# HaokunChen245/FedDAT

Hardware: AMD Instinct MI355X
Metric: VQA samples/sec, ViLT-B/32 dual-adapter local step (higher is better)
Workload: dtype fp16; 1 GPU; configs[1] with fp16 operands (BASELINE.json's configs[1] string says bf16: same operand width and MFMA rate; the bf16 step is in other_operand_format with --full): ViLT-B/32 FedDAT, 1 client per MI355X, fp16 MFMA operands (dynamic loss scale, GradScaler semantics on the device, initial 2^14), fp32 accumulate / masters, batch=32/client, 384x384 synthetic + 40-token questions, MKD on; batch_per_client=32, seq_len=185, clients=1, hip_graph=True, ranks=1, hetero_steps=False

## Files before the change

feddat_amd/csrc/adapter.hip:

```cpp
#include <type_traits>

#include "common.hip.h"

namespace {

constexpr int H = 768, R = 48, NT = 3, KS = H / 32, CT = H / 16;
constexpr int WCOLS = H / 4;
constexpr int WCH = WCOLS / 4;
constexpr int NLD = 16 * WCH / 64;
constexpr int ROWF = 200;
constexpr int STG_WAVE = 16 * ROWF;

struct AdapterLaunch {
    feddat_adapter_seg seg[2];
    int nseg;
    int tiles0;
};

#define FD_COMPILER_FENCE() asm volatile("" ::: "memory")

__device__ __forceinline__ void slice_load(const float* __restrict__ src, int nvalid, int lane, f32x4 (&v)[NLD]) {
#pragma unroll
    for (int j = 0; j < NLD; ++j) {
        const int f = j * 64 + lane, r = f / WCH, c = f - r * WCH;
        const int rr = r < nvalid ? r : nvalid - 1;
        v[j] = *reinterpret_cast<const f32x4*>(src + (size_t)rr * H + c * 4);
    }
}
__device__ __forceinline__ void slice_to_lds(float* stg, int lane, const f32x4 (&v)[NLD]) {
#pragma unroll
    for (int j = 0; j < NLD; ++j) {
        const int f = j * 64 + lane, r = f / WCH, c = f - r * WCH;
        *reinterpret_cast<f32x4*>(stg + r * ROWF + c * 4) = v[j];
    }
}
__device__ __forceinline__ void frags_from_lds(const float* stg, int lane, f32x4 (&keep)[KS / 4][2]) {
    const float* p = stg + (lane & 15) * ROWF + 4 * (lane >> 4);
#pragma unroll
    for (int k = 0; k < KS / 4; ++k) {
        keep[k][0] = *reinterpret_cast<const f32x4*>(p + k * 32);
        keep[k][1] = *reinterpret_cast<const f32x4*>(p + k * 32 + 16);
    }
}
__device__ __forceinline__ void frags_to_lds(float* stg, int lane, const f32x4 (&keep)[KS / 4][2]) {
    float* p = stg + (lane & 15) * ROWF + 4 * (lane >> 4);
#pragma unroll
    for (int k = 0; k < KS / 4; ++k) {
        *reinterpret_cast<f32x4*>(p + k * 32) = keep[k][0];
        *reinterpret_cast<f32x4*>(p + k * 32 + 16) = keep[k][1];
    }
}

template <int NA>
__device__ __forceinline__ void down_proj(const bf16* const* w, int lane, int ks0, f32x4 (&z)[2][NT],
                                          const f32x4 (&keep)[KS / 4][2]) {
#pragma unroll
    for (int k = 0; k < KS / 4; ++k) {
        const int q = ks0 + k;
        const bf16x8 xf = cvt8(keep[k][0], keep[k][1]);
#pragma unroll
        for (int a = 0; a < NA; ++a)
#pragma unroll
            for (int nt = 0; nt < NT; ++nt) {
                const bf16x8 wf = *reinterpret_cast<const bf16x8*>(w[a] + ((nt * KS + q) * 64 + lane) * 8);
                z[a][nt] = mfma16x32(wf, xf, z[a][nt]);
            }
    }
}

__device__ __forceinline__ void load_w48(const bf16* w, int ct, int lane, bf16x8& w01, bf16x8& w2) {
    w01 = *reinterpret_cast<const bf16x8*>(w + (ct * 64 + lane) * 8);
    const bf16x4 c = *reinterpret_cast<const bf16x4*>(w + CT * 64 * 8 + (ct * 64 + lane) * 4);
    w2 = bf16x8{c[0], c[1], c[2], c[3], 0, 0, 0, 0};
}
__device__ __forceinline__ bf16x8 pad8(const f32x4 a) {
    return bf16x8{(bf16)a[0], (bf16)a[1], (bf16)a[2], (bf16)a[3], 0, 0, 0, 0};
}

template <int NS>
__device__ __forceinline__ void ksplit_store(float* stg_all, int wave, int lane, int s, const f32x4 v) {
    reinterpret_cast<f32x4*>(stg_all + wave * STG_WAVE)[s * 64 + lane] = v;
}
template <int NS>
__device__ __forceinline__ f32x4 ksplit_sum(const float* stg_all, int lane, int s) {
    f32x4 t = reinterpret_cast<const f32x4*>(stg_all)[s * 64 + lane];
#pragma unroll
    for (int w = 1; w < 4; ++w) t = t + reinterpret_cast<const f32x4*>(stg_all + w * STG_WAVE)[s * 64 + lane];
    return t;
}

struct LnFuse {
    const float* gamma;
    const float* beta;
    bf16* y16;
    float* stats;
    float eps;
};

template <int NA, bool ZS>
__device__ __forceinline__ void bwd_body(const float* __restrict__ x, const float* __restrict__ dy,
                                         float* __restrict__ dx, bf16* __restrict__ dx16, float* __restrict__ z_out,
                                         float* __restrict__ dz_out, const feddat_adapter_seg& sg, int row0,
                                         float* stg_all, const float* __restrict__ z_saved) {
    const int lane = threadIdx.x & 63, wave = threadIdx.x >> 6;
    const int g = lane >> 4, i16 = lane & 15;
    const int nvalid = (sg.row_end - row0) < 16 ? (sg.row_end - row0) : 16;
    const bool valid = i16 < nvalid;
    const int row = row0 + i16;
    float* stg = stg_all + wave * STG_WAVE;

    const bf16* wd[2] = {(const bf16*)sg.wd[0], (const bf16*)sg.wd[NA - 1]};
    const bf16* wuT[2] = {(const bf16*)sg.wuT[0], (const bf16*)sg.wuT[NA - 1]};
    f32x4 z[2][NT], gr[2][NT];
#pragma unroll
    for (int a = 0; a < 2; ++a)
#pragma unroll
        for (int nt = 0; nt < NT; ++nt) {
            z[a][nt] = f32x4{0.f, 0.f, 0.f, 0.f};
            gr[a][nt] = f32x4{0.f, 0.f, 0.f, 0.f};
        }
    f32x4 dyk[KS / 4][2];
    f32x4 vd[NLD];
    if (ZS) {
        slice_load(dy + (size_t)row0 * H + wave * WCOLS, nvalid, lane, vd);
        const float* zrow = z_saved + (size_t)(valid ? row : row0 + nvalid - 1) * (2 * R) + 4 * g;
#pragma unroll
        for (int a = 0; a < NA; ++a)
#pragma unroll
            for (int nt = 0; nt < NT; ++nt) z[a][nt] = *reinterpret_cast<const f32x4*>(zrow + a * R + nt * 16);
        FD_COMPILER_FENCE();
    } else {
        f32x4 vx[NLD];
        slice_load(x + (size_t)(row0 + sg.x_row_delta) * H + wave * WCOLS, nvalid, lane, vx);
        FD_COMPILER_FENCE();
        f32x4 xk[KS / 4][2];
        slice_to_lds(stg, lane, vx);
        slice_load(dy + (size_t)row0 * H + wave * WCOLS, nvalid, lane, vd);
        FD_COMPILER_FENCE();
        frags_from_lds(stg, lane, xk);
        down_proj<NA>(wd, lane, wave * (KS / 4), z, xk);
    }
    slice_to_lds(stg, lane, vd);
    frags_from_lds(stg, lane, dyk);
    down_proj<NA>(wuT, lane, wave * (KS / 4), gr, dyk);
#pragma unroll
    for (int a = 0; a < NA; ++a)
#pragma unroll
        for (int nt = 0; nt < NT; ++nt) {
            if (!ZS) ksplit_store<2 * NA * NT>(stg_all, wave, lane, a * NT + nt, z[a][nt]);
            ksplit_store<2 * NA * NT>(stg_all, wave, lane, NA * NT + a * NT + nt, gr[a][nt]);
        }
    __syncthreads();

    bf16x8 dzb01[NA], dzb2[NA];
    f32x4 z_keep = f32x4{0.f, 0.f, 0.f, 0.f}, dz_keep = z_keep;
#pragma unroll
    for (int a = 0; a < NA; ++a) {
        const float sc = sg.scale[a];
#pragma unroll
        for (int nt = 0; nt < NT; ++nt) {
            const f32x4 gs = ksplit_sum<2 * NA * NT>(stg_all, lane, NA * NT + a * NT + nt);
            f32x4 zz, dz;
            if (ZS) {
                zz = z[a][nt];
            } else {
                const f32x4 zs = ksplit_sum<2 * NA * NT>(stg_all, lane, a * NT + nt);
                const f32x4 b4 = *reinterpret_cast<const f32x4*>(sg.bd[a] + nt * 16 + 4 * g);
#pragma unroll
                for (int e = 0; e < 4; ++e) zz[e] = fmaxf(zs[e] + b4[e], 0.f);
            }
#pragma unroll
            for (int e = 0; e < 4; ++e) dz[e] = zz[e] > 0.f ? sc * gs[e] : 0.f;
            gr[a][nt] = dz;
            if (a == sg.train_slot && nt == wave) {
                z_keep = zz;
                dz_keep = dz;
            }
        }
        dzb01[a] = cvt8(gr[a][0], gr[a][1]);
        dzb2[a] = pad8(gr[a][2]);
    }
    const bool export_z = sg.train_slot >= 0 && wave < NT && valid && z_out;

    if (dx) {
#pragma unroll
        for (int k = 0; k < CT / 4; ++k) {
            const int ct = wave * (CT / 4) + k;
            f32x4 o = dyk[k >> 1][k & 1];
#pragma unroll
            for (int a = 0; a < NA; ++a) {
                bf16x8 w01, w2;
                load_w48((const bf16*)sg.wdT[a], ct, lane, w01, w2);
                f32x4 y = mfma16x32(w01, dzb01[a], f32x4{0.f, 0.f, 0.f, 0.f});
                y = mfma16x32(w2, dzb2[a], y);
                o = o + y;
            }
            dyk[k >> 1][k & 1] = o;
        }
        __syncthreads();
        frags_to_lds(stg, lane, dyk);
    }
    if (export_z) {
        *reinterpret_cast<f32x4*>(z_out + (size_t)row * R + wave * 16 + 4 * g) = z_keep;
        *reinterpret_cast<f32x4*>(dz_out + (size_t)row * R + wave * 16 + 4 * g) = dz_keep;
    }
    if (!dx) return;
    float* orow = dx + (size_t)row0 * H + wave * WCOLS;
    f32x4 v[NLD];
#pragma unroll
    for (int j = 0; j < NLD; ++j) {
        const int f = j * 64 + lane, r = f / WCH, c = f - r * WCH;
        v[j] = *reinterpret_cast<const f32x4*>(stg + r * ROWF + c * 4);
    }
#pragma unroll
    for (int j = 0; j < NLD; ++j) {
        const int f = j * 64 + lane, r = f / WCH, c = f - r * WCH;
        if (r < nvalid) *reinterpret_cast<f32x4*>(orow + (size_t)r * H + c * 4) = v[j];
    }
    if (dx16) {
        bf16* brow = dx16 + (size_t)row0 * H + wave * WCOLS;
#pragma unroll
        for (int j = 0; j < NLD; ++j) {
            const int f = j * 64 + lane, r = f / WCH, c = f - r * WCH;
            if (r < nvalid) *reinterpret_cast<bf16x4*>(brow + (size_t)r * H + c * 4) = cvt4(v[j]);
        }
    }
}

template <bool ZS>
__global__ __launch_bounds__(256, 2) void adapter_bwd_kernel(const float* __restrict__ x, const float* __restrict__ dy,
                                                          float* __restrict__ dx, bf16* __restrict__ dx16,
                                                          float* __restrict__ z_out, float* __restrict__ dz_out,
                                                          AdapterLaunch L, const float* __restrict__ z_saved) {
    __shared__ __attribute__((aligned(16))) float stg[4 * STG_WAVE];
    const int tile = blockIdx.x;
    const int s = tile < L.tiles0 ? 0 : 1;
    const int t = s ? tile - L.tiles0 : tile;
    const feddat_adapter_seg& sg = L.seg[s];
    const int row0 = sg.row_begin + t * 16;
    if (sg.n_adapters == 2) bwd_body<2, ZS>(x, dy, dx, dx16, z_out, dz_out, sg, row0, stg, z_saved);
    else bwd_body<1, ZS>(x, dy, dx, dx16, z_out, dz_out, sg, row0, stg, z_saved);
}

constexpr int ROWT = H + 8;
constexpr int TILE_F = 16 * ROWT;
constexpr int KSPL_F = 4 * 6 * 64 * 4;
constexpr int ZT_F = 16 * 2 * R;

struct WsLaunch {
    AdapterLaunch a;
    int g0;
    int dbg;
};

#define FD_WAIT_VM0() asm volatile("s_waitcnt vmcnt(0)" ::: "memory")
constexpr int WS_WEIGHT_LOADS_PER_ADAPTER = NT * (KS / 4) + CT / 4 + 2 * (CT / 8);
static_assert(WS_WEIGHT_LOADS_PER_ADAPTER == 42, "ws_load_weights changed: re-derive the counted wait");
template <int NA>
__device__ __forceinline__ void ws_wait_tile0(bool has_tile1) {
    constexpr int behind = NA * WS_WEIGHT_LOADS_PER_ADAPTER + 12;
    constexpr int cnt = behind < 63 ? behind : 63;
    if (has_tile1) asm volatile("s_waitcnt vmcnt(%0)" ::"n"(cnt) : "memory");
    else FD_WAIT_VM0();
}

__device__ __forceinline__ void ws_dma16(const float* g, const float* lds_dst) {
    const unsigned a = __builtin_amdgcn_readfirstlane((unsigned)(uintptr_t)LDS_PTR(lds_dst));
    asm volatile("s_mov_b32 m0, %1\n\ts_nop 0\n\tglobal_load_lds_dwordx4 %0, off" : : "v"(g), "s"(a) : "memory");
}
__device__ __forceinline__ void ws_tile_dma(const float* __restrict__ src, int nvalid, float* buf, int wave, int lane) {
#pragma unroll
    for (int j = 0; j < 12; ++j) {
        const int r = wave * 4 + j / 3, part = j % 3;
        const int rr = r < nvalid ? r : nvalid - 1;
        ws_dma16(src + (size_t)rr * H + part * 256 + lane * 4, buf + r * ROWT + part * 256);
    }
}
__device__ __forceinline__ void ws_frags_from_lds(const float* buf, int wave, int lane, f32x4 (&keep)[KS / 4][2]) {
    const float* p = buf + (lane & 15) * ROWT + wave * WCOLS + 4 * (lane >> 4);
#pragma unroll
    for (int k = 0; k < KS / 4; ++k) {
        keep[k][0] = *reinterpret_cast<const f32x4*>(p + k * 32);
        keep[k][1] = *reinterpret_cast<const f32x4*>(p + k * 32 + 16);
    }
}
__device__ __forceinline__ void ws_frags_to_lds(float* buf, int wave, int lane, const f32x4 (&keep)[KS / 4][2]) {
    float* p = buf + (lane & 15) * ROWT + wave * WCOLS + 4 * (lane >> 4);
#pragma unroll
    for (int k = 0; k < KS / 4; ++k) {
        *reinterpret_cast<f32x4*>(p + k * 32) = keep[k][0];
        *reinterpret_cast<f32x4*>(p + k * 32 + 16) = keep[k][1];
    }
}

template <int NA>
struct WsWeights {
    bf16x8 dn[NA][NT][KS / 4];
    bf16x8 up01[NA][CT / 4];
    bf16x8 up2[NA][CT / 8];
};
template <int NA>
__device__ __forceinline__ void ws_load_weights(WsWeights<NA>& W, const void* const* dn, const void* const* up, int wave,
                                                int lane) {
#pragma unroll
    for (int a = 0; a < NA; ++a) {
        const bf16* d = (const bf16*)dn[a];
        const bf16* u = (const bf16*)up[a];
#pragma unroll
        for (int nt = 0; nt < NT; ++nt)
#pragma unroll
            for (int k = 0; k < KS / 4; ++k)
                W.dn[a][nt][k] = *reinterpret_cast<const bf16x8*>(d + ((nt * KS + wave * (KS / 4) + k) * 64 + lane) * 8);
#pragma unroll
        for (int k = 0; k < CT / 4; ++k) {
            const int ct = wave * (CT / 4) + k;
            W.up01[a][k] = *reinterpret_cast<const bf16x8*>(u + (ct * 64 + lane) * 8);
        }
#pragma unroll
        for (int p = 0; p < CT / 8; ++p) {
            const int ct = wave * (CT / 4) + 2 * p;
            const bf16x4 lo = *reinterpret_cast<const bf16x4*>(u + CT * 64 * 8 + (ct * 64 + lane) * 4);
            const bf16x4 hi = *reinterpret_cast<const bf16x4*>(u + CT * 64 * 8 + ((ct + 1) * 64 + lane) * 4);
            W.up2[a][p] = bf16x8{lo[0], lo[1], lo[2], lo[3], hi[0], hi[1], hi[2], hi[3]};
        }
    }
}
__device__ __forceinline__ bf16x8 pad8hi(const f32x4 a) {
    return bf16x8{0, 0, 0, 0, (bf16)a[0], (bf16)a[1], (bf16)a[2], (bf16)a[3]};
}

__device__ __forceinline__ void ws_walk(const WsLaunch& L, int& s, int& t0, int& tstep, int& ntiles) {
    const int b = blockIdx.x;
    s = b < L.g0 ? 0 : 1;
    t0 = s ? b - L.g0 : b;
    tstep = s ? (int)gridDim.x - L.g0 : L.g0;
    const feddat_adapter_seg& sg = L.a.seg[s];
    ntiles = (sg.row_end - sg.row_begin + 15) / 16;
}

template <int NA>
__device__ __forceinline__ void ws_fwd_body(const float* __restrict__ x, float* __restrict__ out,
                                            const feddat_adapter_seg& sg, int t0, int tstep, int ntiles, float* smem,
                                            const LnFuse& ln, float* __restrict__ z_save, const int dbg) {
    const int lane = threadIdx.x & 63, wave = threadIdx.x >> 6;
    const int g = lane >> 4, i16 = lane & 15;
    float* kspl = smem + 2 * TILE_F;
    float* lnred = kspl + KSPL_F;
    float* sbu = lnred + 256;
    float* sbd = sbu + 2 * H;
    float* sgam = sbd + 128;
    float* sbet = sgam + H;
    if (t0 >= ntiles) return;

    auto tile_dma = [&](int p) {
        const int t = t0 + p * tstep;
        if (t < ntiles && !(p && (dbg & 4))) {
            const int row0 = sg.row_begin + t * 16;
            const int nvalid = (sg.row_end - row0) < 16 ? (sg.row_end - row0) : 16;
            ws_tile_dma(x + (size_t)(row0 + sg.x_row_delta) * H, nvalid, smem + p * TILE_F, wave, lane);
        }
    };
    for (int i = threadIdx.x; i < NA * H; i += 256) sbu[i] = sg.bu[i / H][i % H];
    if (threadIdx.x < NA * R) sbd[(threadIdx.x / R) * 64 + threadIdx.x % R] = sg.bd[threadIdx.x / R][threadIdx.x % R];
    if (ln.gamma)
        for (int i = threadIdx.x; i < H; i += 256) {
            sgam[i] = ln.gamma[i];
            sbet[i] = ln.beta[i];
        }
    float sc[NA];
#pragma unroll
    for (int a = 0; a < NA; ++a) sc[a] = sg.scale[a];
    tile_dma(0);
    WsWeights<NA> W;
    ws_load_weights<NA>(W, sg.wd, sg.wu, wave, lane);
    tile_dma(1);
    ws_wait_tile0<NA>(!(dbg & 4) && t0 + tstep < ntiles);
    __syncthreads();

    int cur = 0;
    for (int t = t0; t < ntiles; t += tstep, cur ^= 1) {
        const int row0 = sg.row_begin + t * 16;
        const int nvalid = (sg.row_end - row0) < 16 ? (sg.row_end - row0) : 16;
        float* buf = smem + cur * TILE_F;

        f32x4 z_keep[NA];
        float mean = 0.f, rstd = 0.f;
#pragma unroll
        for (int a = 0; a < NA; ++a) z_keep[a] = f32x4{0.f, 0.f, 0.f, 0.f};
        if (!(dbg & 2)) {
        const float* frag = buf + i16 * ROWT + wave * WCOLS + 4 * g;
        f32x4 z[NA][NT];
#pragma unroll
        for (int a = 0; a < NA; ++a)
#pragma unroll
            for (int nt = 0; nt < NT; ++nt) z[a][nt] = f32x4{0.f, 0.f, 0.f, 0.f};
#pragma unroll
        for (int k = 0; k < KS / 4; ++k) {
            const bf16x8 xf = cvt8(*reinterpret_cast<const f32x4*>(frag + k * 32),
                                   *reinterpret_cast<const f32x4*>(frag + k * 32 + 16));
#pragma unroll
            for (int a = 0; a < NA; ++a)
#pragma unroll
                for (int nt = 0; nt < NT; ++nt) z[a][nt] = mfma16x32(W.dn[a][nt][k], xf, z[a][nt]);
        }
#pragma unroll
        for (int a = 0; a < NA; ++a)
#pragma unroll
            for (int nt = 0; nt < NT; ++nt)
                reinterpret_cast<f32x4*>(kspl)[(wave * 6 + a * NT + nt) * 64 + lane] = z[a][nt];
        __syncthreads();
        bf16x8 zb01[NA], zb2[NA][2];
#pragma unroll
        for (int a = 0; a < NA; ++a) {
#pragma unroll
            for (int nt = 0; nt < NT; ++nt) {
                f32x4 tsum = reinterpret_cast<const f32x4*>(kspl)[(a * NT + nt) * 64 + lane];
#pragma unroll
                for (int w = 1; w < 4; ++w) tsum = tsum + reinterpret_cast<const f32x4*>(kspl)[(w * 6 + a * NT + nt) * 64 + lane];
                const f32x4 b4 = *reinterpret_cast<const f32x4*>(sbd + a * 64 + nt * 16 + 4 * g);
#pragma unroll
                for (int e = 0; e < 4; ++e) z[a][nt][e] = fmaxf(tsum[e] + b4[e], 0.f);
                if (nt == wave) z_keep[a] = z[a][nt];
            }
            zb01[a] = cvt8(z[a][0], z[a][1]);
            zb2[a][0] = pad8(z[a][2]);
            zb2[a][1] = pad8hi(z[a][2]);
        }

        f32x4 xk[KS / 4][2];
#pragma unroll
        for (int k = 0; k < CT / 4; ++k) {
            const int c = (wave * (CT / 4) + k) * 16 + 4 * g;
            f32x4 o = *reinterpret_cast<const f32x4*>(frag + k * 16);
#pragma unroll
            for (int a = 0; a < NA; ++a) {
                f32x4 y = mfma16x32(W.up01[a][k], zb01[a], f32x4{0.f, 0.f, 0.f, 0.f});
                y = mfma16x32(W.up2[a][k >> 1], zb2[a][k & 1], y);
                const f32x4 bu4 = *reinterpret_cast<const f32x4*>(sbu + a * H + c);
#pragma unroll
                for (int e = 0; e < 4; ++e) o[e] += sc[a] * (y[e] + bu4[e]);
            }
            xk[k >> 1][k & 1] = o;
        }

        if (ln.gamma) {
            float s1 = 0.f;
#pragma unroll
            for (int k = 0; k < CT / 4; ++k) {
                const f32x4 o = xk[k >> 1][k & 1];
                s1 += (o[0] + o[1]) + (o[2] + o[3]);
            }
            s1 += __shfl_xor(s1, 16, 64);
            s1 += __shfl_xor(s1, 32, 64);
            const float mw = s1 * (1.0f / WCOLS);
            float s2 = 0.f;
#pragma unroll
            for (int k = 0; k < CT / 4; ++k)
#pragma unroll
                for (int e = 0; e < 4; ++e) {
                    const float d = xk[k >> 1][k & 1][e] - mw;
                    s2 += d * d;
                }
            s2 += __shfl_xor(s2, 16, 64);
            s2 += __shfl_xor(s2, 32, 64);
            if (g == 0) {
                lnred[wave * 32 + 2 * i16] = mw;
                lnred[wave * 32 + 2 * i16 + 1] = s2;
            }
            __syncthreads();
            const float m0 = lnred[2 * i16], m1 = lnred[32 + 2 * i16], m2 = lnred[64 + 2 * i16], m3 = lnred[96 + 2 * i16];
            mean = ((m0 + m1) + (m2 + m3)) * 0.25f;
            const float q0 = m0 - mean, q1 = m1 - mean, q2 = m2 - mean, q3 = m3 - mean;
            const float M2 = ((lnred[2 * i16 + 1] + lnred[32 + 2 * i16 + 1]) + (lnred[64 + 2 * i16 + 1] + lnred[96 + 2 * i16 + 1])) +
                             (float)WCOLS * ((q0 * q0 + q1 * q1) + (q2 * q2 + q3 * q3));
            rstd = rsqrtf(M2 * (1.0f / H) + ln.eps);
            if (g == 0) {
                lnred[128 + wave * 32 + 2 * i16] = mean;
                lnred[128 + wave * 32 + 2 * i16 + 1] = rstd;
            }
        }

        ws_frags_to_lds(buf, wave, lane, xk);
        }
        float* orow = out + (size_t)row0 * H + wave * WCOLS;
        const float* srow = buf + wave * WCOLS;
        f32x4 v[NLD];
#pragma unroll
        for (int j = 0; j < NLD; ++j) {
            const int r = 4 * (j / 3) + g, c = 16 * (j % 3) + i16;
            v[j] = *reinterpret_cast<const f32x4*>(srow + r * ROWT + c * 4);
        }
        FD_WAIT_VM0();
        const bool st_on = !(dbg & 1);
        auto emit = [&](auto full_tag) {
            constexpr bool FULL = decltype(full_tag)::value;
            if (z_save && wave < NT && (FULL || i16 < nvalid)) {
#pragma unroll
                for (int a = 0; a < NA; ++a)
                    *reinterpret_cast<f32x4*>(z_save + (size_t)(row0 + i16) * (2 * R) + a * R + wave * 16 + 4 * g) = z_keep[a];
            }
#pragma unroll
            for (int j = 0; j < NLD; ++j) {
                const int r = 4 * (j / 3) + g, c = 16 * (j % 3) + i16;
                if (FULL || r < nvalid) *reinterpret_cast<f32x4*>(orow + (size_t)r * H + c * 4) = v[j];
            }
            if (ln.gamma) {
                bf16* yrow = ln.y16 + (size_t)row0 * H + wave * WCOLS;
#pragma unroll
                for (int j = 0; j < NLD; ++j) {
                    const int r = 4 * (j / 3) + g, c = 16 * (j % 3) + i16;
                    const float m = lnred[128 + wave * 32 + 2 * r], rs = lnred[128 + wave * 32 + 2 * r + 1];
                    const f32x4 gm = *reinterpret_cast<const f32x4*>(sgam + wave * WCOLS + c * 4);
                    const f32x4 bt = *reinterpret_cast<const f32x4*>(sbet + wave * WCOLS + c * 4);
                    f32x4 y;
#pragma unroll
                    for (int e = 0; e < 4; ++e) y[e] = (v[j][e] - m) * rs * gm[e] + bt[e];
                    if (FULL || r < nvalid) *reinterpret_cast<bf16x4*>(yrow + (size_t)r * H + c * 4) = cvt4(y);
                }
                if (wave == 0 && g == 0 && (FULL || i16 < nvalid) && ln.stats) {
                    ln.stats[2 * (size_t)(row0 + i16)] = mean;
                    ln.stats[2 * (size_t)(row0 + i16) + 1] = rstd;
                }
            }
        };
        if (st_on) {
            if (nvalid == 16) emit(std::true_type{});
            else emit(std::false_type{});
        }
        __syncthreads();
        if (t + 2 * tstep < ntiles && !(dbg & 4)) {
            const int rn = sg.row_begin + (t + 2 * tstep) * 16;
            const int nv = (sg.row_end - rn) < 16 ? (sg.row_end - rn) : 16;
            ws_tile_dma(x + (size_t)(rn + sg.x_row_delta) * H, nv, buf, wave, lane);
        }
    }
}

constexpr int WS_FWD_LDS = (2 * TILE_F + KSPL_F + 256 + 2 * H + 128 + 2 * H) * 4;

__global__ __launch_bounds__(256, 1) void adapter_fwd_ws_kernel(const float* __restrict__ x, float* __restrict__ out,
                                                                WsLaunch L, LnFuse ln, float* __restrict__ z_save) {
    extern __shared__ __attribute__((aligned(16))) float ws_smem[];
    int s, t0, tstep, ntiles;
    ws_walk(L, s, t0, tstep, ntiles);
    const feddat_adapter_seg& sg = L.a.seg[s];
    if (sg.n_adapters == 2) ws_fwd_body<2>(x, out, sg, t0, tstep, ntiles, ws_smem, ln, z_save, FD_ABL(L.dbg));
    else ws_fwd_body<1>(x, out, sg, t0, tstep, ntiles, ws_smem, ln, z_save, FD_ABL(L.dbg));
}


__device__ __forceinline__ void ws_ztile_dma(const float* __restrict__ zs, int nvalid, float* dst, int wave, int lane) {
#pragma unroll
    for (int j = 0; j < 2; ++j) {
        const int piece = wave + 4 * j;
        if (piece < 6) {
            const int fo = piece * 256 + lane * 4, r = fo / (2 * R), c = fo - r * (2 * R);
            const int rr = r < nvalid ? r : nvalid - 1;
            ws_dma16(zs + (size_t)rr * (2 * R) + c, dst + piece * 256);
        }
    }
}

template <int NA, bool Q8>
__device__ __forceinline__ void ws_bwd_body(const float* __restrict__ dy, float* __restrict__ dx, bf16* __restrict__ dx16,
                                            float* __restrict__ z_out, float* __restrict__ dz_out,
                                            const feddat_adapter_seg& sg, int t0, int tstep, int ntiles, float* smem,
                                            const float* __restrict__ z_saved, const int dbg,
                                            unsigned char* __restrict__ dx8, float* __restrict__ dx8_scale) {
    const int lane = threadIdx.x & 63, wave = threadIdx.x >> 6;
    const int g = lane >> 4, i16 = lane & 15;
    float* kspl = smem + 2 * TILE_F;
    float* ztile = kspl + KSPL_F;
    float* amred = ztile + 2 * ZT_F;
    if (t0 >= ntiles) return;
    auto tile_dma = [&](int p) {
        const int t = t0 + p * tstep;
        if (t < ntiles && !(p && (dbg & 4))) {
            const int row0 = sg.row_begin + t * 16;
            const int nvalid = (sg.row_end - row0) < 16 ? (sg.row_end - row0) : 16;
            ws_tile_dma(dy + (size_t)row0 * H, nvalid, smem + p * TILE_F, wave, lane);
            ws_ztile_dma(z_saved + (size_t)row0 * (2 * R), nvalid, ztile + p * ZT_F, wave, lane);
        }
    };
    if (Q8) {
#pragma unroll
        for (int p = 0; p < 2; ++p) {
            const int t = t0 + p * tstep;
            if (t < ntiles && !(p && (dbg & 4))) {
                const int row0 = sg.row_begin + t * 16;
                const int nvalid = (sg.row_end - row0) < 16 ? (sg.row_end - row0) : 16;
                ws_tile_dma(dy + (size_t)row0 * H, nvalid, smem + p * TILE_F, wave, lane);
                ws_ztile_dma(z_saved + (size_t)row0 * (2 * R), nvalid, ztile + p * ZT_F, wave, lane);
            }
        }
    } else {
        tile_dma(0);
    }
    WsWeights<NA> W;
    ws_load_weights<NA>(W, sg.wuT, sg.wdT, wave, lane);
    if (!Q8) tile_dma(1);
    float sc[NA];
#pragma unroll
    for (int a = 0; a < NA; ++a) sc[a] = sg.scale[a];
    const int train_slot = sg.train_slot;
    const bool exp_z = train_slot >= 0 && wave < NT && z_out;
    ws_wait_tile0<NA>(!Q8 && !(dbg & 4) && t0 + tstep < ntiles);
    __syncthreads();

    int cur = 0;
    for (int t = t0; t < ntiles; t += tstep, cur ^= 1) {
        const int row0 = sg.row_begin + t * 16;
        const int nvalid = (sg.row_end - row0) < 16 ? (sg.row_end - row0) : 16;
        float* buf = smem + cur * TILE_F;
        float* zt = ztile + cur * ZT_F;

        f32x4 z_keep = f32x4{0.f, 0.f, 0.f, 0.f}, dz_keep = z_keep;
        if (!(dbg & 2)) {
        const float* frag = buf + i16 * ROWT + wave * WCOLS + 4 * g;
        f32x4 gr[NA][NT];
#pragma unroll
        for (int a = 0; a < NA; ++a)
#pragma unroll
            for (int nt = 0; nt < NT; ++nt) gr[a][nt] = f32x4{0.f, 0.f, 0.f, 0.f};
#pragma unroll
        for (int k = 0; k < KS / 4; ++k) {
            const bf16x8 df = cvt8(*reinterpret_cast<const f32x4*>(frag + k * 32),
                                   *reinterpret_cast<const f32x4*>(frag + k * 32 + 16));
#pragma unroll
            for (int a = 0; a < NA; ++a)
#pragma unroll
                for (int nt = 0; nt < NT; ++nt) gr[a][nt] = mfma16x32(W.dn[a][nt][k], df, gr[a][nt]);
        }
#pragma unroll
        for (int a = 0; a < NA; ++a)
#pragma unroll
            for (int nt = 0; nt < NT; ++nt)
                reinterpret_cast<f32x4*>(kspl)[(wave * 6 + a * NT + nt) * 64 + lane] = gr[a][nt];
        __syncthreads();

        bf16x8 dzb01[NA], dzb2[NA][2];
#pragma unroll
        for (int a = 0; a < NA; ++a) {
#pragma unroll
            for (int nt = 0; nt < NT; ++nt) {
                f32x4 gs = reinterpret_cast<const f32x4*>(kspl)[(a * NT + nt) * 64 + lane];
#pragma unroll
                for (int w = 1; w < 4; ++w) gs = gs + reinterpret_cast<const f32x4*>(kspl)[(w * 6 + a * NT + nt) * 64 + lane];
                const f32x4 zz = *reinterpret_cast<const f32x4*>(zt + i16 * (2 * R) + a * R + nt * 16 + 4 * g);
                f32x4 dz;
#pragma unroll
                for (int e = 0; e < 4; ++e) dz[e] = zz[e] > 0.f ? sc[a] * gs[e] : 0.f;
                gr[a][nt] = dz;
                if (a == train_slot && nt == wave) {
                    z_keep = zz;
                    dz_keep = dz;
                }
            }
            dzb01[a] = cvt8(gr[a][0], gr[a][1]);
            dzb2[a][0] = pad8(gr[a][2]);
            dzb2[a][1] = pad8hi(gr[a][2]);
        }
        if (dx) {
#pragma unroll
            for (int k = 0; k < CT / 4; ++k) {
                f32x4 o = *reinterpret_cast<const f32x4*>(frag + k * 16);
#pragma unroll
                for (int a = 0; a < NA; ++a) {
                    f32x4 y = mfma16x32(W.up01[a][k], dzb01[a], f32x4{0.f, 0.f, 0.f, 0.f});
                    y = mfma16x32(W.up2[a][k >> 1], dzb2[a][k & 1], y);
                    o = o + y;
                }
                *reinterpret_cast<f32x4*>(buf + i16 * ROWT + wave * WCOLS + 4 * g + k * 16) = o;
            }
        }
        }
        f32x4 v[NLD];
        if (dx) {
            const float* srow = buf + wave * WCOLS;
#pragma unroll
            for (int j = 0; j < NLD; ++j) {
                const int r = 4 * (j / 3) + g, c = 16 * (j % 3) + i16;
                v[j] = *reinterpret_cast<const f32x4*>(srow + r * ROWT + c * 4);
            }
        }
        float sc8[4] = {1.f, 1.f, 1.f, 1.f};
        if (Q8 && dx && dx8) {
#pragma unroll
            for (int q = 0; q < 4; ++q) {
                float am = 0.f;
#pragma unroll
                for (int jj = 0; jj < 3; ++jj)
#pragma unroll
                    for (int e = 0; e < 4; ++e) am = fmaxf(am, fabsf(v[3 * q + jj][e]));
                am = fmaxf(am, __shfl_xor(am, 1, 64));
                am = fmaxf(am, __shfl_xor(am, 2, 64));
                am = fmaxf(am, __shfl_xor(am, 4, 64));
                am = fmaxf(am, __shfl_xor(am, 8, 64));
                if (i16 == 0) amred[wave * 16 + 4 * q + g] = am;
            }
            __syncthreads();
#pragma unroll
            for (int q = 0; q < 4; ++q) {
                const int r = 4 * q + g;
                const float am = fmaxf(fmaxf(amred[r], amred[16 + r]), fmaxf(amred[32 + r], amred[48 + r]));
                sc8[q] = am > 0.f ? am * (1.0f / 448.0f) : 1.0f;
            }
        }
        FD_WAIT_VM0();
        const bool st_on = !(dbg & 1);
        auto emit = [&](auto full_tag) {
            constexpr bool FULL = decltype(full_tag)::value;
            if (exp_z && (FULL || i16 < nvalid)) {
                *reinterpret_cast<f32x4*>(z_out + (size_t)(row0 + i16) * R + wave * 16 + 4 * g) = z_keep;
                *reinterpret_cast<f32x4*>(dz_out + (size_t)(row0 + i16) * R + wave * 16 + 4 * g) = dz_keep;
            }
            if (dx) {
                float* orow = dx + (size_t)row0 * H + wave * WCOLS;
#pragma unroll
                for (int j = 0; j < NLD; ++j) {
                    const int r = 4 * (j / 3) + g, c = 16 * (j % 3) + i16;
                    if (FULL || r < nvalid) *reinterpret_cast<f32x4*>(orow + (size_t)r * H + c * 4) = v[j];
                }
                if (dx16) {
                    bf16* brow = dx16 + (size_t)row0 * H + wave * WCOLS;
#pragma unroll
                    for (int j = 0; j < NLD; ++j) {
                        const int r = 4 * (j / 3) + g, c = 16 * (j % 3) + i16;
                        if (FULL || r < nvalid) *reinterpret_cast<bf16x4*>(brow + (size_t)r * H + c * 4) = cvt4(v[j]);
                    }
                }
                if (Q8 && dx8) {
                    unsigned char* qrow = dx8 + (size_t)row0 * H + wave * WCOLS;
#pragma unroll
                    for (int j = 0; j < NLD; ++j) {
                        const int r = 4 * (j / 3) + g, c = 16 * (j % 3) + i16;
                        const float inv = 1.0f / sc8[j / 3];
                        int pk = __builtin_amdgcn_cvt_pk_fp8_f32(v[j][0] * inv, v[j][1] * inv, 0, false);
                        pk = __builtin_amdgcn_cvt_pk_fp8_f32(v[j][2] * inv, v[j][3] * inv, pk, true);
                        if (FULL || r < nvalid) *reinterpret_cast<int*>(qrow + (size_t)r * H + c * 4) = pk;
                    }
                    if (wave == 0 && i16 == 0) {
#pragma unroll
                        for (int q = 0; q < 4; ++q)
                            if (FULL || 4 * q + g < nvalid) dx8_scale[row0 + 4 * q + g] = sc8[q];
                    }
                }
            }
        };
        if (st_on) {
            if (nvalid == 16) emit(std::true_type{});
            else emit(std::false_type{});
        }
        __syncthreads();
        if (t + 2 * tstep < ntiles && !(dbg & 4)) {
            const int rn = sg.row_begin + (t + 2 * tstep) * 16;
            const int nv = (sg.row_end - rn) < 16 ? (sg.row_end - rn) : 16;
            ws_tile_dma(dy + (size_t)rn * H, nv, buf, wave, lane);
            ws_ztile_dma(z_saved + (size_t)rn * (2 * R), nv, zt, wave, lane);
        }
    }
}

constexpr int WS_BWD_LDS = (2 * TILE_F + KSPL_F + 2 * ZT_F + 64) * 4;

template <bool Q8>
__global__ __launch_bounds__(256, 1) void adapter_bwd_ws_kernel(const float* __restrict__ dy, float* __restrict__ dx,
                                                                bf16* __restrict__ dx16, float* __restrict__ z_out,
                                                                float* __restrict__ dz_out, WsLaunch L,
                                                                const float* __restrict__ z_saved,
                                                                unsigned char* __restrict__ dx8, float* __restrict__ dx8_scale) {
    extern __shared__ __attribute__((aligned(16))) float ws_smem[];
    int s, t0, tstep, ntiles;
    ws_walk(L, s, t0, tstep, ntiles);
    const feddat_adapter_seg& sg = L.a.seg[s];
    if (sg.n_adapters == 2) ws_bwd_body<2, Q8>(dy, dx, dx16, z_out, dz_out, sg, t0, tstep, ntiles, ws_smem, z_saved, FD_ABL(L.dbg), dx8,
                                               dx8_scale);
    else ws_bwd_body<1, Q8>(dy, dx, dx16, z_out, dz_out, sg, t0, tstep, ntiles, ws_smem, z_saved, FD_ABL(L.dbg), dx8, dx8_scale);
}

int ws_plan(const AdapterLaunch& A, int tiles, WsLaunch& L, int& grid) {
    int n_cu = 0;
    const int rc = fd_device_cus(&n_cu);
    if (rc) return rc;
    L.a = A;
    L.dbg = FD_ABL((fd_debug_flags() >> 24) & 7);
    const int t0 = A.tiles0, t1 = tiles - A.tiles0;
    grid = tiles < n_cu ? tiles : n_cu;
    if (t1 == 0) L.g0 = grid;
    else if (t0 == 0) L.g0 = 0;
    else {
        int g0 = (int)(((long)grid * t0 + tiles / 2) / tiles);
        g0 = g0 < 1 ? 1 : (g0 > grid - 1 ? grid - 1 : g0);
        L.g0 = g0;
    }
    return FEDDAT_OK;
}


__global__ __launch_bounds__(256) void adapter_pack_kernel(const float* __restrict__ wd, const float* __restrict__ wu,
                                                           bf16* __restrict__ wd16, bf16* __restrict__ wdT16,
                                                           bf16* __restrict__ wu16, bf16* __restrict__ wuT16,
                                                           long stride32, long stride16) {
    wd += blockIdx.y * stride32; wu += blockIdx.y * stride32;
    wd16 += blockIdx.y * stride16; wdT16 += blockIdx.y * stride16;
    wu16 += blockIdx.y * stride16; wuT16 += blockIdx.y * stride16;
    const int i = blockIdx.x * 256 + threadIdx.x;
    if (i >= R * H) return;
    auto down_idx = [](int r, int c) {
        const int pc = (c & ~31) + (((c & 15) >> 2) << 3) + (((c >> 4) & 1) << 2) + (c & 3);
        const int q = pc >> 5, g = (pc & 31) >> 3, j = pc & 7;
        return ((((r >> 4) * KS + q) * 64 + g * 16 + (r & 15)) << 3) + j;
    };
    auto up_idx = [](int c, int r) {
        const int ct = c >> 4, i16 = c & 15, seg = r >> 4, g = (r & 15) >> 2, e = r & 3;
        const int lane = g * 16 + i16;
        return seg < 2 ? ((ct * 64 + lane) << 3) + seg * 4 + e : CT * 64 * 8 + ((ct * 64 + lane) << 2) + e;
    };
    {
        const int r = i / H, c = i - r * H;
        const bf16 v = (bf16)wd[i];
        wd16[down_idx(r, c)] = v;
        wdT16[up_idx(c, r)] = v;
    }
    {
        const int c = i / R, r = i - c * R;
        const bf16 v = (bf16)wu[i];
        wu16[up_idx(c, r)] = v;
        wuT16[down_idx(r, c)] = v;
    }
}

int prep_launch(const feddat_adapter_seg* segs, int nseg, int T, AdapterLaunch& L, int& tiles, bool bwd) {
    if (!segs || nseg < 1 || nseg > 2) return FEDDAT_EINVAL;
    L.nseg = nseg;
    tiles = 0;
    for (int s = 0; s < nseg; ++s) {
        const feddat_adapter_seg& sg = segs[s];
        if (sg.row_begin < 0 || sg.row_end > T || sg.row_end < sg.row_begin) return FEDDAT_EINVAL;
        if (sg.row_begin + sg.x_row_delta < 0 || sg.row_end + sg.x_row_delta > T) return FEDDAT_EINVAL;
        if (sg.n_adapters != 1 && sg.n_adapters != 2) return FEDDAT_EINVAL;
        if (bwd && (sg.train_slot < -1 || sg.train_slot >= sg.n_adapters)) return FEDDAT_EINVAL;
        for (int a = 0; a < sg.n_adapters; ++a) {
            if (!sg.wd[a] || !sg.wu[a] || !sg.bd[a] || !sg.bu[a]) return FEDDAT_EINVAL;
            if (bwd && (!sg.wdT[a] || !sg.wuT[a])) return FEDDAT_EINVAL;
        }
        L.seg[s] = sg;
        const int t = (sg.row_end - sg.row_begin + 15) / 16;
        if (s == 0) L.tiles0 = t;
        tiles += t;
    }
    if (nseg == 1) L.seg[1] = L.seg[0];
    return FEDDAT_OK;
}

int dbg_extra_lds() { return FD_ABL(((fd_debug_flags() >> 16) & 0xff) * 1024); }

int ws_launch_fwd(const float* x, float* out, const AdapterLaunch& A, int tiles, const LnFuse& ln, float* z_save,
                  hipStream_t stream) {
    WsLaunch W;
    int grid;
    int rc = ws_plan(A, tiles, W, grid);
    if (rc) return rc;
    rc = fd_set_max_lds((const void*)adapter_fwd_ws_kernel, WS_FWD_LDS);
    if (rc) return rc;
    hipLaunchKernelGGL(adapter_fwd_ws_kernel, dim3(grid), dim3(256), WS_FWD_LDS, stream, x, out, W, ln, z_save);
    FD_LAUNCH_RET();
}

}

extern "C" int feddat_adapter_fwd(const float* x, float* out, int T, int Hd, int r, const feddat_adapter_seg* segs,
                                  int nseg, float* z_save, hipStream_t stream) {
    FD_CHECK_ARG(x && out && T > 0 && Hd == H && r == R);
    AdapterLaunch L;
    int tiles;
    const int rc = prep_launch(segs, nseg, T, L, tiles, false);
    if (rc) return rc;
    if (tiles == 0) return FEDDAT_OK;
    return ws_launch_fwd(x, out, L, tiles, LnFuse{nullptr, nullptr, nullptr, nullptr, 0.f}, z_save, stream);
}

extern "C" int feddat_adapter_fwd_ln(const float* x, float* out, int T, int Hd, int r, const feddat_adapter_seg* segs,
                                     int nseg, const float* ln_gamma, const float* ln_beta, float eps, void* y_bf16,
                                     float* stats, float* z_save, hipStream_t stream) {
    FD_CHECK_ARG(x && out && T > 0 && Hd == H && r == R && ln_gamma && ln_beta && y_bf16);
    AdapterLaunch L;
    int tiles;
    const int rc = prep_launch(segs, nseg, T, L, tiles, false);
    if (rc) return rc;
    if (tiles == 0) return FEDDAT_OK;
    return ws_launch_fwd(x, out, L, tiles, LnFuse{ln_gamma, ln_beta, (bf16*)y_bf16, stats, eps}, z_save, stream);
}

static int adapter_bwd_launch(const float* x, const float* z_saved, const float* dy, float* dx, void* dx_bf16, void* dx_fp8,
                              float* dx_scale, float* z_out, float* dz_out, int T, int Hd, int r,
                              const feddat_adapter_seg* segs, int nseg, hipStream_t stream) {
    FD_CHECK_ARG((x || z_saved) && dy && (dx || z_out) && T > 0 && Hd == H && r == R);
    FD_CHECK_ARG((z_out == nullptr) == (dz_out == nullptr));
    FD_CHECK_ARG((dx_fp8 == nullptr) == (dx_scale == nullptr) && (!dx_fp8 || (z_saved && dx)));
    AdapterLaunch L;
    int tiles;
    const int rc = prep_launch(segs, nseg, T, L, tiles, true);
    if (rc) return rc;
    if (tiles == 0) return FEDDAT_OK;
    if (z_saved) {
        WsLaunch W;
        int grid;
        const int rc2 = ws_plan(L, tiles, W, grid);
        if (rc2) return rc2;
        if (dx_fp8) {
            const int rc3 = fd_set_max_lds((const void*)adapter_bwd_ws_kernel<true>, WS_BWD_LDS);
            if (rc3) return rc3;
            hipLaunchKernelGGL(adapter_bwd_ws_kernel<true>, dim3(grid), dim3(256), WS_BWD_LDS, stream, dy, dx, (bf16*)dx_bf16,
                               z_out, dz_out, W, z_saved, (unsigned char*)dx_fp8, dx_scale);
        } else {
            const int rc3 = fd_set_max_lds((const void*)adapter_bwd_ws_kernel<false>, WS_BWD_LDS);
            if (rc3) return rc3;
            hipLaunchKernelGGL(adapter_bwd_ws_kernel<false>, dim3(grid), dim3(256), WS_BWD_LDS, stream, dy, dx, (bf16*)dx_bf16,
                               z_out, dz_out, W, z_saved, (unsigned char*)nullptr, (float*)nullptr);
        }
    } else {
        hipLaunchKernelGGL(adapter_bwd_kernel<false>, dim3(tiles), dim3(256), dbg_extra_lds(), stream, x, dy, dx,
                           (bf16*)dx_bf16, z_out, dz_out, L, z_saved);
    }
    FD_LAUNCH_RET();
}

extern "C" int feddat_adapter_bwd(const float* x, const float* z_saved, const float* dy, float* dx, void* dx_bf16,
                                  float* z_out, float* dz_out, int T, int Hd, int r, const feddat_adapter_seg* segs,
                                  int nseg, hipStream_t stream) {
    return adapter_bwd_launch(x, z_saved, dy, dx, dx_bf16, nullptr, nullptr, z_out, dz_out, T, Hd, r, segs, nseg, stream);
}

extern "C" int feddat_adapter_bwd_fp8(const float* z_saved, const float* dy, float* dx, void* dx_fp8, float* dx_scale,
                                      float* z_out, float* dz_out, int T, int Hd, int r, const feddat_adapter_seg* segs,
                                      int nseg, hipStream_t stream) {
    FD_CHECK_ARG(z_saved && dx && dx_fp8 && dx_scale);
    return adapter_bwd_launch(nullptr, z_saved, dy, dx, nullptr, dx_fp8, dx_scale, z_out, dz_out, T, Hd, r, segs, nseg, stream);
}

extern "C" int feddat_adapter_pack(const float* wd, const float* wu, void* wd_bf16, void* wdT_bf16, void* wu_bf16,
                                   void* wuT_bf16, int Hd, int r, hipStream_t stream) {
    FD_CHECK_ARG(wd && wu && wd_bf16 && wdT_bf16 && wu_bf16 && wuT_bf16 && Hd == H && r == R);
    hipLaunchKernelGGL(adapter_pack_kernel, dim3((R * H + 255) / 256), dim3(256), 0, stream, wd, wu, (bf16*)wd_bf16,
                       (bf16*)wdT_bf16, (bf16*)wu_bf16, (bf16*)wuT_bf16, 0L, 0L);
    FD_LAUNCH_RET();
}

extern "C" int feddat_adapter_pack_strided(const float* wd, const float* wu, long stride_f32, void* wd_bf16,
                                           void* wdT_bf16, void* wu_bf16, void* wuT_bf16, long stride_bf16, int n,
                                           int Hd, int r, hipStream_t stream) {
    FD_CHECK_ARG(wd && wu && wd_bf16 && wdT_bf16 && wu_bf16 && wuT_bf16 && Hd == H && r == R);
    FD_CHECK_ARG(n > 0 && n <= 65535 && stride_f32 >= 0 && stride_bf16 >= 0);
    hipLaunchKernelGGL(adapter_pack_kernel, dim3((R * H + 255) / 256, n), dim3(256), 0, stream, wd, wu, (bf16*)wd_bf16,
                       (bf16*)wdT_bf16, (bf16*)wu_bf16, (bf16*)wuT_bf16, stride_f32, stride_bf16);
    FD_LAUNCH_RET();
}
```

Baseline: 4532 samples/s.

## Triple-buffer adapter forward tiles and interleave previous tile's stores with MFMA compute

The forward adapter kernel moves from two tile buffers to three. The global stores of the previous tile's output and its LayerNorm bf16 output are deferred and interleaved, piece by piece, between the MFMA steps of the current tile, using sched_barrier so they overlap compute instead of running as a serial epilogue. Up-bias, gamma and beta now sit in registers (the bias is spread with DPP row broadcasts) instead of being staged in LDS. The k-split reduction reuses one smaller LDS slice per adapter, and LN and ablation become template parameters. This raises register pressure and LDS footprint, and adds an extra __syncthreads per adapter in the reduction.

```diff
diff --git a/feddat_amd/csrc/adapter.hip b/feddat_amd/csrc/adapter.hip
--- a/feddat_amd/csrc/adapter.hip
+++ b/feddat_amd/csrc/adapter.hip
@@ -1,4 +1,5 @@
 #include <type_traits>
+#include <utility>
 
 #include "common.hip.h"
 
@@ -338,18 +339,34 @@
     ntiles = (sg.row_end - sg.row_begin + 15) / 16;
 }
 
-template <int NA>
+template <int N>
+__device__ __forceinline__ float ws_row_bcast(float v) {
+    return __builtin_bit_cast(float, __builtin_amdgcn_update_dpp(0, __builtin_bit_cast(int, v), 0x150 + N, 0xf, 0xf, false));
+}
+template <class F, int... I>
+__device__ __forceinline__ void ws_static_for_impl(F&& f, std::integer_sequence<int, I...>) {
+    (f(std::integral_constant<int, I>{}), ...);
+}
+template <int N, class F>
+__device__ __forceinline__ void ws_static_for(F&& f) {
+    ws_static_for_impl(f, std::make_integer_sequence<int, N>{});
+}
+
+constexpr int KSPL1_F = 4 * NT * 64 * 4;
+constexpr int LNRED_F = 128 + 2 * 128;
+constexpr int WS_FWD_LDS = (3 * TILE_F + KSPL1_F + LNRED_F + 128) * 4;
+static_assert(WS_FWD_LDS <= 160 * 1024, "adapter_fwd_ws_kernel: three tile buffers no longer fit the CU's 160 KiB of LDS");
+
+template <int NA, bool LN, bool ABL>
 __device__ __forceinline__ void ws_fwd_body(const float* __restrict__ x, float* __restrict__ out,
                                             const feddat_adapter_seg& sg, int t0, int tstep, int ntiles, float* smem,
-                                            const LnFuse& ln, float* __restrict__ z_save, const int dbg) {
+                                            const LnFuse& ln, float* __restrict__ z_save, const int dbg_flags) {
+    const int dbg = ABL ? dbg_flags : 0;
     const int lane = threadIdx.x & 63, wave = threadIdx.x >> 6;
     const int g = lane >> 4, i16 = lane & 15;
-    float* kspl = smem + 2 * TILE_F;
-    float* lnred = kspl + KSPL_F;
-    float* sbu = lnred + 256;
-    float* sbd = sbu + 2 * H;
-    float* sgam = sbd + 128;
-    float* sbet = sgam + H;
+    float* kspl = smem + 3 * TILE_F;
+    float* lnred = kspl + KSPL1_F;
+    float* sbd = lnred + LNRED_F;
     if (t0 >= ntiles) return;
 
     auto tile_dma = [&](int p) {
@@ -360,13 +377,21 @@
             ws_tile_dma(x + (size_t)(row0 + sg.x_row_delta) * H, nvalid, smem + p * TILE_F, wave, lane);
         }
     };
-    for (int i = threadIdx.x; i < NA * H; i += 256) sbu[i] = sg.bu[i / H][i % H];
     if (threadIdx.x < NA * R) sbd[(threadIdx.x / R) * 64 + threadIdx.x % R] = sg.bd[threadIdx.x / R][threadIdx.x % R];
-    if (ln.gamma)
-        for (int i = threadIdx.x; i < H; i += 256) {
-            sgam[i] = ln.gamma[i];
-            sbet[i] = ln.beta[i];
-        }
+    float but[NA][3];
+#pragma unroll
+    for (int a = 0; a < NA; ++a)
+#pragma unroll
+        for (int m = 0; m < 3; ++m) but[a][m] = sg.bu[a][wave * WCOLS + (4 * m + (i16 >> 2)) * 16 + 4 * g + (i16 & 3)];
+    f32x4 gm[3], bt[3];
+#pragma unroll
+    for (int p = 0; p < 3; ++p) {
+        gm[p] = bt[p] = f32x4{0.f, 0.f, 0.f, 0.f};
+        if (LN) {
+            gm[p] = *reinterpret_cast<const f32x4*>(ln.gamma + wave * WCOLS + (16 * p + i16) * 4);
+            bt[p] = *reinterpret_cast<const f32x4*>(ln.beta + wave * WCOLS + (16 * p + i16) * 4);
+        }
+    }
     float sc[NA];
 #pragma unroll
     for (int a = 0; a < NA; ++a) sc[a] = sg.scale[a];
@@ -377,17 +402,56 @@
     ws_wait_tile0<NA>(!(dbg & 4) && t0 + tstep < ntiles);
     __syncthreads();
 
-    int cur = 0;
-    for (int t = t0; t < ntiles; t += tstep, cur ^= 1) {
-        const int row0 = sg.row_begin + t * 16;
-        const int nvalid = (sg.row_end - row0) < 16 ? (sg.row_end - row0) : 16;
-        float* buf = smem + cur * TILE_F;
-
-        f32x4 z_keep[NA];
-        float mean = 0.f, rstd = 0.f;
-#pragma unroll
-        for (int a = 0; a < NA; ++a) z_keep[a] = f32x4{0.f, 0.f, 0.f, 0.f};
-        if (!(dbg & 2)) {
+    f32x4 z_def[NA];
+#pragma unroll
+    for (int a = 0; a < NA; ++a) z_def[a] = f32x4{0.f, 0.f, 0.f, 0.f};
+    int drow0 = 0;
+    const bool st_on = !(dbg & 1);
+    auto piece = [&](auto full_tag, int j, const float* dbuf, const float* lnd, int nv) __attribute__((always_inline)) {
+        constexpr bool FULL = decltype(full_tag)::value;
+        const int r = 4 * (j / 3) + g, c = 16 * (j % 3) + i16;
+        const f32x4 v = *reinterpret_cast<const f32x4*>(dbuf + wave * WCOLS + r * ROWT + c * 4);
+        if (FULL || r < nv) *reinterpret_cast<f32x4*>(out + (size_t)(drow0 + r) * H + wave * WCOLS + c * 4) = v;
+        if (LN) {
+            const float m = lnd[wave * 32 + 2 * r], rs = lnd[wave * 32 + 2 * r + 1];
+            const f32x4 gmj = gm[j % 3], btj = bt[j % 3];
+            f32x4 y;
+#pragma unroll
+            for (int e = 0; e < 4; ++e) y[e] = (v[e] - m) * rs * gmj[e] + btj[e];
+            if (FULL || r < nv) *reinterpret_cast<bf16x4*>(ln.y16 + (size_t)(drow0 + r) * H + wave * WCOLS + c * 4) = cvt4(y);
+        }
+    };
+    auto head = [&](auto full_tag, const float* lnd, int nv) __attribute__((always_inline)) {
+        constexpr bool FULL = decltype(full_tag)::value;
+        if (z_save && wave < NT && (FULL || i16 < nv)) {
+#pragma unroll
+            for (int a = 0; a < NA; ++a)
+                *reinterpret_cast<f32x4*>(z_save + (size_t)(drow0 + i16) * (2 * R) + a * R + wave * 16 + 4 * g) = z_def[a];
+        }
+        if (LN && wave == 0 && g == 0 && (FULL || i16 < nv) && ln.stats) {
+            ln.stats[2 * (size_t)(drow0 + i16)] = lnd[2 * i16];
+            ln.stats[2 * (size_t)(drow0 + i16) + 1] = lnd[2 * i16 + 1];
+        }
+    };
+
+    auto tile = [&](auto defer_tag, float* buf, const float* dbuf, float* lnc, const float* lnd) __attribute__((always_inline)) {
+        constexpr bool DEFER = decltype(defer_tag)::value;
+        auto dpiece = [&](int j) __attribute__((always_inline)) {
+            if (DEFER) {
+                piece(std::true_type{}, j, dbuf, lnd, 16);
+                __builtin_amdgcn_sched_barrier(0);
+            }
+        };
+        if (dbg & 2) {
+            if (DEFER) {
+                head(std::true_type{}, lnd, 16);
+#pragma unroll
+                for (int j = 0; j < NLD; ++j) piece(std::true_type{}, j, dbuf, lnd, 16);
+            }
+            return;
+        }
+        if (DEFER) head(std::true_type{}, lnd, 16);
+
         const float* frag = buf + i16 * ROWT + wave * WCOLS + 4 * g;
         f32x4 z[NA][NT];
 #pragma unroll
@@ -402,48 +466,53 @@
             for (int a = 0; a < NA; ++a)
 #pragma unroll
                 for (int nt = 0; nt < NT; ++nt) z[a][nt] = mfma16x32(W.dn[a][nt][k], xf, z[a][nt]);
-        }
-#pragma unroll
-        for (int a = 0; a < NA; ++a)
-#pragma unroll
-            for (int nt = 0; nt < NT; ++nt)
-                reinterpret_cast<f32x4*>(kspl)[(wave * 6 + a * NT + nt) * 64 + lane] = z[a][nt];
-        __syncthreads();
+            if (!(k & 1)) dpiece(k >> 1);
+        }
         bf16x8 zb01[NA], zb2[NA][2];
 #pragma unroll
         for (int a = 0; a < NA; ++a) {
+            if (a) __syncthreads();
+#pragma unroll
+            for (int nt = 0; nt < NT; ++nt) reinterpret_cast<f32x4*>(kspl)[(wave * NT + nt) * 64 + lane] = z[a][nt];
+            __syncthreads();
 #pragma unroll
             for (int nt = 0; nt < NT; ++nt) {
-                f32x4 tsum = reinterpret_cast<const f32x4*>(kspl)[(a * NT + nt) * 64 + lane];
-#pragma unroll
-                for (int w = 1; w < 4; ++w) tsum = tsum + reinterpret_cast<const f32x4*>(kspl)[(w * 6 + a * NT + nt) * 64 + lane];
+                f32x4 tsum = reinterpret_cast<const f32x4*>(kspl)[nt * 64 + lane];
+#pragma unroll
+                for (int w = 1; w < 4; ++w) tsum = tsum + reinterpret_cast<const f32x4*>(kspl)[(w * NT + nt) * 64 + lane];
                 const f32x4 b4 = *reinterpret_cast<const f32x4*>(sbd + a * 64 + nt * 16 + 4 * g);
 #pragma unroll
                 for (int e = 0; e < 4; ++e) z[a][nt][e] = fmaxf(tsum[e] + b4[e], 0.f);
-                if (nt == wave) z_keep[a] = z[a][nt];
+                if (nt == wave) z_def[a] = z[a][nt];
             }
             zb01[a] = cvt8(z[a][0], z[a][1]);
             zb2[a][0] = pad8(z[a][2]);
             zb2[a][1] = pad8hi(z[a][2]);
-        }
+            dpiece(3 + a);
+        }
+        if (NA == 1) dpiece(4);
 
         f32x4 xk[KS / 4][2];
-#pragma unroll
-        for (int k = 0; k < CT / 4; ++k) {
-            const int c = (wave * (CT / 4) + k) * 16 + 4 * g;
+        ws_static_for<CT / 4>([&](auto kc) __attribute__((always_inline)) {
+            constexpr int k = decltype(kc)::value;
             f32x4 o = *reinterpret_cast<const f32x4*>(frag + k * 16);
 #pragma unroll
             for (int a = 0; a < NA; ++a) {
                 f32x4 y = mfma16x32(W.up01[a][k], zb01[a], f32x4{0.f, 0.f, 0.f, 0.f});
                 y = mfma16x32(W.up2[a][k >> 1], zb2[a][k & 1], y);
-                const f32x4 bu4 = *reinterpret_cast<const f32x4*>(sbu + a * H + c);
+                float bm = but[a][k >> 2];
+                asm volatile("" : "+v"(bm));
+                const f32x4 bu4 = f32x4{ws_row_bcast<4 * (k & 3)>(bm), ws_row_bcast<4 * (k & 3) + 1>(bm),
+                                        ws_row_bcast<4 * (k & 3) + 2>(bm), ws_row_bcast<4 * (k & 3) + 3>(bm)};
 #pragma unroll
                 for (int e = 0; e < 4; ++e) o[e] += sc[a] * (y[e] + bu4[e]);
             }
             xk[k >> 1][k & 1] = o;
-        }
-
-        if (ln.gamma) {
+            if (!(k & 1)) dpiece(5 + (k >> 1));
+        });
+        dpiece(11);
+
+        if (LN) {
             float s1 = 0.f;
 #pragma unroll
             for (int k = 0; k < CT / 4; ++k) {
@@ -469,74 +538,59 @@
             }
             __syncthreads();
             const float m0 = lnred[2 * i16], m1 = lnred[32 + 2 * i16], m2 = lnred[64 + 2 * i16], m3 = lnred[96 + 2 * i16];
-            mean = ((m0 + m1) + (m2 + m3)) * 0.25f;
+            const float mean = ((m0 + m1) + (m2 + m3)) * 0.25f;
             const float q0 = m0 - mean, q1 = m1 - mean, q2 = m2 - mean, q3 = m3 - mean;
             const float M2 = ((lnred[2 * i16 + 1] + lnred[32 + 2 * i16 + 1]) + (lnred[64 + 2 * i16 + 1] + lnred[96 + 2 * i16 + 1])) +
                              (float)WCOLS * ((q0 * q0 + q1 * q1) + (q2 * q2 + q3 * q3));
-            rstd = rsqrtf(M2 * (1.0f / H) + ln.eps);
+            const float rstd = rsqrtf(M2 * (1.0f / H) + ln.eps);
             if (g == 0) {
-                lnred[128 + wave * 32 + 2 * i16] = mean;
-                lnred[128 + wave * 32 + 2 * i16 + 1] = rstd;
+                lnc[wave * 32 + 2 * i16] = mean;
+                lnc[wave * 32 + 2 * i16 + 1] = rstd;
             }
         }
 
         ws_frags_to_lds(buf, wave, lane, xk);
-        }
-        float* orow = out + (size_t)row0 * H + wave * WCOLS;
-        const float* srow = buf + wave * WCOLS;
-        f32x4 v[NLD];
-#pragma unroll
-        for (int j = 0; j < NLD; ++j) {
-            const int r = 4 * (j / 3) + g, c = 16 * (j % 3) + i16;
-            v[j] = *reinterpret_cast<const f32x4*>(srow + r * ROWT + c * 4);
-        }
+    };
+
+    int cur = 0, prv = 2, par = 0;
+    auto step = [&](auto defer_tag, int t) __attribute__((always_inline)) {
+        float* buf = smem + cur * TILE_F;
+        const float* dbuf = smem + prv * TILE_F;
+        float* lnc = lnred + 128 + par * 128;
+        const float* lnd = lnred + 128 + (par ^ 1) * 128;
+        if (ABL && !st_on) tile(std::false_type{}, buf, dbuf, lnc, lnd);
+        else tile(defer_tag, buf, dbuf, lnc, lnd);
         FD_WAIT_VM0();
-        const bool st_on = !(dbg & 1);
-        auto emit = [&](auto full_tag) {
-            constexpr bool FULL = decltype(full_tag)::value;
-            if (z_save && wave < NT && (FULL || i16 < nvalid)) {
-#pragma unroll
-                for (int a = 0; a < NA; ++a)
-                    *reinterpret_cast<f32x4*>(z_save + (size_t)(row0 + i16) * (2 * R) + a * R + wave * 16 + 4 * g) = z_keep[a];
-            }
-#pragma unroll
-            for (int j = 0; j < NLD; ++j) {
-                const int r = 4 * (j / 3) + g, c = 16 * (j % 3) + i16;
-                if (FULL || r < nvalid) *reinterpret_cast<f32x4*>(orow + (size_t)r * H + c * 4) = v[j];
-            }
-            if (ln.gamma) {
-                bf16* yrow = ln.y16 + (size_t)row0 * H + wave * WCOLS;
-#pragma unroll
-                for (int j = 0; j < NLD; ++j) {
-                    const int r = 4 * (j / 3) + g, c = 16 * (j % 3) + i16;
-                    const float m = lnred[128 + wave * 32 + 2 * r], rs = lnred[128 + wave * 32 + 2 * r + 1];
-                    const f32x4 gm = *reinterpret_cast<const f32x4*>(sgam + wave * WCOLS + c * 4);
-                    const f32x4 bt = *reinterpret_cast<const f32x4*>(sbet + wave * WCOLS + c * 4);
-                    f32x4 y;
-#pragma unroll
-                    for (int e = 0; e < 4; ++e) y[e] = (v[j][e] - m) * rs * gm[e] + bt[e];
-                    if (FULL || r < nvalid) *reinterpret_cast<bf16x4*>(yrow + (size_t)r * H + c * 4) = cvt4(y);
-                }
-                if (wave == 0 && g == 0 && (FULL || i16 < nvalid) && ln.stats) {
-                    ln.stats[2 * (size_t)(row0 + i16)] = mean;
-                    ln.stats[2 * (size_t)(row0 + i16) + 1] = rstd;
-                }
-            }
-        };
-        if (st_on) {
-            if (nvalid == 16) emit(std::true_type{});
-            else emit(std::false_type{});
-        }
         __syncthreads();
         if (t + 2 * tstep < ntiles && !(dbg & 4)) {
             const int rn = sg.row_begin + (t + 2 * tstep) * 16;
             const int nv = (sg.row_end - rn) < 16 ? (sg.row_end - rn) : 16;
-            ws_tile_dma(x + (size_t)(rn + sg.x_row_delta) * H, nv, buf, wave, lane);
-        }
-    }
-}
-
-constexpr int WS_FWD_LDS = (2 * TILE_F + KSPL_F + 256 + 2 * H + 128 + 2 * H) * 4;
+            ws_tile_dma(x + (size_t)(rn + sg.x_row_delta) * H, nv, smem + prv * TILE_F, wave, lane);
+        }
+        drow0 = sg.row_begin + t * 16;
+        const int nxt = 3 - cur - prv;
+        prv = cur;
+        cur = nxt;
+        par ^= 1;
+    };
+    step(std::false_type{}, t0);
+    for (int t = t0 + tstep; t < ntiles; t += tstep) step(std::true_type{}, t);
+
+    if (st_on) {
+        const float* dbuf = smem + prv * TILE_F;
+        const float* lnd = lnred + 128 + (par ^ 1) * 128;
+        const int nv = (sg.row_end - drow0) < 16 ? (sg.row_end - drow0) : 16;
+        if (nv == 16) {
+            head(std::true_type{}, lnd, 16);
+#pragma unroll
+            for (int j = 0; j < NLD; ++j) piece(std::true_type{}, j, dbuf, lnd, 16);
+        } else {
+            head(std::false_type{}, lnd, nv);
+#pragma unroll
+            for (int j = 0; j < NLD; ++j) piece(std::false_type{}, j, dbuf, lnd, nv);
+        }
+    }
+}
 
 __global__ __launch_bounds__(256, 1) void adapter_fwd_ws_kernel(const float* __restrict__ x, float* __restrict__ out,
                                                                 WsLaunch L, LnFuse ln, float* __restrict__ z_save) {
@@ -544,8 +598,19 @@
     int s, t0, tstep, ntiles;
     ws_walk(L, s, t0, tstep, ntiles);
     const feddat_adapter_seg& sg = L.a.seg[s];
-    if (sg.n_adapters == 2) ws_fwd_body<2>(x, out, sg, t0, tstep, ntiles, ws_smem, ln, z_save, FD_ABL(L.dbg));
-    else ws_fwd_body<1>(x, out, sg, t0, tstep, ntiles, ws_smem, ln, z_save, FD_ABL(L.dbg));
+    auto run = [&](auto abl_tag) __attribute__((always_inline)) {
+        constexpr bool ABL = decltype(abl_tag)::value;
+        const int dbg = FD_ABL(L.dbg);
+        if (ln.gamma) {
+            if (sg.n_adapters == 2) ws_fwd_body<2, true, ABL>(x, out, sg, t0, tstep, ntiles, ws_smem, ln, z_save, dbg);
+            else ws_fwd_body<1, true, ABL>(x, out, sg, t0, tstep, ntiles, ws_smem, ln, z_save, dbg);
+        } else {
+            if (sg.n_adapters == 2) ws_fwd_body<2, false, ABL>(x, out, sg, t0, tstep, ntiles, ws_smem, ln, z_save, dbg);
+            else ws_fwd_body<1, false, ABL>(x, out, sg, t0, tstep, ntiles, ws_smem, ln, z_save, dbg);
+        }
+    };
+    if (FD_ABL(L.dbg) == 0) run(std::false_type{});
+    else run(std::true_type{});
 }
 
 
```

Measured after the change: 4541 samples/s (median of 3 runs). No clear change (+0.2%).
